# RaghuvirJonnagiri/LatticeBoltzmannSimulations

Hardware: AMD Instinct MI355X
Metric: MLUPS (million lattice updates/sec) D2Q9 MRT cavity (higher is better)
Workload: dtype f32

## Files before the change

### latticeboltzmannsimulations_amd/csrc/lbm_stream.hpp

```cpp
#pragma once
#include "lbm_kernels.hpp"

constexpr int ST_WAVES = 16;
constexpr int ST_NT = ST_WAVES * 64;
constexpr int ST_MAX_S = ST_WAVES / 2;
constexpr int ST_LDS_BYTES = ST_WAVES * 9 * 1024;

__device__ __forceinline__ int dpp_from_lower(int v) { return __builtin_amdgcn_update_dpp(v, v, 0x138, 0xf, 0xf, false); }
__device__ __forceinline__ int dpp_from_upper(int v) { return __builtin_amdgcn_update_dpp(v, v, 0x130, 0xf, 0xf, false); }
__device__ __forceinline__ float lane_lower(float v) { return __builtin_bit_cast(float, dpp_from_lower(__builtin_bit_cast(int, v))); }
__device__ __forceinline__ float lane_upper(float v) { return __builtin_bit_cast(float, dpp_from_upper(__builtin_bit_cast(int, v))); }
__device__ __forceinline__ double lane_lower(double v) {
    const long long b = __builtin_bit_cast(long long, v);
    const unsigned lo = (unsigned)dpp_from_lower((int)(unsigned)b), hi = (unsigned)dpp_from_lower((int)(unsigned)(b >> 32));
    return __builtin_bit_cast(double, (long long)(((unsigned long long)hi << 32) | lo));
}
__device__ __forceinline__ double lane_upper(double v) {
    const long long b = __builtin_bit_cast(long long, v);
    const unsigned lo = (unsigned)dpp_from_upper((int)(unsigned)b), hi = (unsigned)dpp_from_upper((int)(unsigned)(b >> 32));
    return __builtin_bit_cast(double, (long long)(((unsigned long long)hi << 32) | lo));
}

__device__ __forceinline__ float lane_lower_e(float v, float edge) {
    return __builtin_bit_cast(float, __builtin_amdgcn_update_dpp(__builtin_bit_cast(int, edge), __builtin_bit_cast(int, v), 0x138, 0xf, 0xf, false));
}
__device__ __forceinline__ float lane_upper_e(float v, float edge) {
    return __builtin_bit_cast(float, __builtin_amdgcn_update_dpp(__builtin_bit_cast(int, edge), __builtin_bit_cast(int, v), 0x130, 0xf, 0xf, false));
}
__device__ __forceinline__ double lane_lower_e(double v, double edge) {
    const long long b = __builtin_bit_cast(long long, v), e = __builtin_bit_cast(long long, edge);
    const unsigned lo = (unsigned)__builtin_amdgcn_update_dpp((int)(unsigned)e, (int)(unsigned)b, 0x138, 0xf, 0xf, false);
    const unsigned hi = (unsigned)__builtin_amdgcn_update_dpp((int)(unsigned)(e >> 32), (int)(unsigned)(b >> 32), 0x138, 0xf, 0xf, false);
    return __builtin_bit_cast(double, (long long)(((unsigned long long)hi << 32) | lo));
}
__device__ __forceinline__ double lane_upper_e(double v, double edge) {
    const long long b = __builtin_bit_cast(long long, v), e = __builtin_bit_cast(long long, edge);
    const unsigned lo = (unsigned)__builtin_amdgcn_update_dpp((int)(unsigned)e, (int)(unsigned)b, 0x130, 0xf, 0xf, false);
    const unsigned hi = (unsigned)__builtin_amdgcn_update_dpp((int)(unsigned)(e >> 32), (int)(unsigned)(b >> 32), 0x130, 0xf, 0xf, false);
    return __builtin_bit_cast(double, (long long)(((unsigned long long)hi << 32) | lo));
}
template <typename R, int V>
__device__ __forceinline__ typename VecT<R, V>::type shift_from_lower_e(typename VecT<R, V>::type own, R edge) {
    typename VecT<R, V>::type r;
    r[0] = lane_lower_e(own[V - 1], edge);
#pragma unroll
    for (int c = 1; c < V; ++c) r[c] = own[c - 1];
    return r;
}
template <typename R, int V>
__device__ __forceinline__ typename VecT<R, V>::type shift_from_upper_e(typename VecT<R, V>::type own, R edge) {
    typename VecT<R, V>::type r;
#pragma unroll
    for (int c = 0; c < V - 1; ++c) r[c] = own[c + 1];
    r[V - 1] = lane_upper_e(own[0], edge);
    return r;
}

template <typename R, int V>
__device__ __forceinline__ typename VecT<R, V>::type shift_from_lower(typename VecT<R, V>::type own) {
    typename VecT<R, V>::type r;
    r[0] = lane_lower(own[V - 1]);
#pragma unroll
    for (int c = 1; c < V; ++c) r[c] = own[c - 1];
    return r;
}
template <typename R, int V>
__device__ __forceinline__ typename VecT<R, V>::type shift_from_upper(typename VecT<R, V>::type own) {
    typename VecT<R, V>::type r;
#pragma unroll
    for (int c = 0; c < V - 1; ++c) r[c] = own[c + 1];
    r[V - 1] = lane_upper(own[0]);
    return r;
}

__host__ __device__ constexpr int stream_rim(int S, int V) { return (S + V - 1) / V * V; }

#ifdef LBM_EXPERIMENT_NO_BARRIER
__device__ __forceinline__ void lds_barrier() { asm volatile("s_waitcnt lgkmcnt(0)" ::: "memory"); }
#else
__device__ __forceinline__ void lds_barrier() { asm volatile("s_waitcnt lgkmcnt(0)\n\ts_barrier" ::: "memory"); }
#endif

template <typename R, int V, bool PROM = false>
__device__ __forceinline__ void wall_row_rules(typename VecT<R, V>::type (&in)[Q], typename VecT<R, V>::type& rw, bool lid, R uLB, bool wl, bool wr,
                                               R& kl, R& kr) {
    typedef typename VecT<R, V>::type T;
    if (lid) {
        const T ux = T(uLB), uy = T((R)0);
        const T cq = (R)1.5 * (ux * ux + uy * uy);
        auto fek = [&](int k) {
            const T cu = cu_of<T>(k, ux, uy);
            if constexpr (PROM) {
                const T rt = rw * weight<R>(k), usqr = ux * ux + uy * uy;
                T fe;
#pragma unroll
                for (int c = 0; c < V; ++c) fe[c] = feq_prom(rt[c], cu[c], usqr[c]);
                return fe;
            } else {
                return (rw * weight<R>(k)) * ((((R)1. + (R)3.0 * cu) + ((R)4.5 * cu) * cu) - cq);
            }
        };
        if (wl) {
            const R g7 = kl;
            in[1][0] = (fek(1)[0] - fek(3)[0]) + in[3][0];
            in[5][0] = (fek(5)[0] - fek(7)[0]) + g7;
            in[8][0] = (fek(8)[0] - fek(6)[0]) + in[6][0];
        }
        if (wr) {
            const R g8 = kr;
            in[3][V - 1] = (-fek(1)[V - 1] + fek(3)[V - 1]) + in[1][V - 1];
            in[6][V - 1] = (-fek(8)[V - 1] + fek(6)[V - 1]) + g8;
            in[7][V - 1] = (-fek(5)[V - 1] + fek(7)[V - 1]) + in[5][V - 1];
        }
        in[4] = (-fek(2) + fek(4)) + in[2];
        in[7] = (-fek(5) + fek(7)) + in[5];
        in[8] = (-fek(6) + fek(8)) + in[6];
        if (wl) kl = in[7][0];
        if (wr) kr = in[8][V - 1];
        rw = ((in[0] + in[1]) + in[3]) + (R)2. * ((in[2] + in[5]) + in[6]);
    } else {
        if (wl) {
            const R g6 = kl;
            in[1][0] = (R)0 + in[3][0];
            in[5][0] = (R)0 + in[7][0];
            in[8][0] = (R)0 + g6;
        }
        if (wr) {
            const R g5 = kr;
            in[3][V - 1] = (R)0 + in[1][V - 1];
            in[6][V - 1] = (R)0 + in[8][V - 1];
            in[7][V - 1] = (R)0 + g5;
        }
        in[2] = (R)0 + in[4];
        in[5] = (R)0 + in[7];
        in[6] = (R)0 + in[8];
        if (wl) kl = in[6][0];
        if (wr) kr = in[5][V - 1];
    }
}

template <typename R, int V, bool WALLS>
__device__ __forceinline__ void build_in(typename VecT<R, V>::type (&in)[Q], typename VecT<R, V>::type o0, typename VecT<R, V>::type o1,
                                         typename VecT<R, V>::type o3, typename VecT<R, V>::type u2, typename VecT<R, V>::type u5,
                                         typename VecT<R, V>::type u6, typename VecT<R, V>::type d4, typename VecT<R, V>::type d7,
                                         typename VecT<R, V>::type d8) {
    in[0] = o0;
    in[2] = u2;
    in[4] = d4;
    if (WALLS) {
        in[1] = shift_from_lower_e<R, V>(o1, (R)0 + o3[1]);
        in[5] = shift_from_lower_e<R, V>(u5, (R)0 + d7[1]);
        in[8] = shift_from_lower_e<R, V>(d8, (R)0 + u6[1]);
        in[3] = shift_from_upper_e<R, V>(o3, (R)0 + o1[V - 2]);
        in[6] = shift_from_upper_e<R, V>(u6, (R)0 + d8[V - 2]);
        in[7] = shift_from_upper_e<R, V>(d7, (R)0 + u5[V - 2]);
    } else {
        in[1] = shift_from_lower<R, V>(o1);
        in[5] = shift_from_lower<R, V>(u5);
        in[8] = shift_from_lower<R, V>(d8);
        in[3] = shift_from_upper<R, V>(o3);
        in[6] = shift_from_upper<R, V>(u6);
        in[7] = shift_from_upper<R, V>(d7);
    }
}

template <typename R, int COLL, bool TURB, bool WALLS = false, bool SLAB = false>
__device__ __forceinline__ void stream_segment(const R* __restrict__ src, R* __restrict__ dst, const Geo& geo, const Relax<R>& w, R* __restrict__ lds,
                                               int S, int xs, int ya, int yb, int xe, int own_lo = 0, int own_hi = 0) {
    constexpr int V = 16 / (int)sizeof(R), ROW = 64 * V;
    typedef typename VecT<R, V>::type T;
    const int wv = __builtin_amdgcn_readfirstlane((int)(threadIdx.x >> 6)), lane = threadIdx.x & 63;
    const int q = ((wv & 7) << 1) | (wv >> 3);
    const int RV = stream_rim(S, V) / V;
    const bool wall_lo = WALLS && (!SLAB || geo.y0 == 0), wall_hi = WALLS && (!SLAB || geo.y0 + geo.ny == geo.NY);
    const int y_first = wall_lo ? max(ya - (S - 1), 0) : ya - (S - 1);
    const int y_end = wall_hi ? min(yb + (S - 1), geo.ny) : yb + (S - 1);
    const int y_lid = wall_lo ? 0 : -(1 << 30), y_bot = wall_hi ? geo.ny - 1 : -(1 << 30);
    const int nb = y_end - y_first;
    const int x0 = xs + lane * V;
    const bool lane_in = x0 < geo.nx;
    const bool lane_out = WALLS ? (x0 >= own_lo && x0 < own_hi) : (lane >= RV && lane < 64 - RV && x0 < xe);
    const bool wl = WALLS && x0 == 0, wr = WALLS && x0 + V == geo.nx;
    const bool side_strip = WALLS && (xs == 0 || xs + ROW >= geo.nx);
    const bool narrow = WALLS && xs + ROW > geo.nx;
    R* const slot_mine = lds + (q * 9) * ROW;
    R* const up_mine = slot_mine + lane * V;
    const R* const up_below = lds + (((q + 1) & (ST_WAVES - 1)) * 9) * ROW + lane * V;
    const R* const down_above = lds + (((q + ST_WAVES - 1) & (ST_WAVES - 1)) * 9 + 3) * ROW + lane * V;

    T in[Q], outv[Q], hq, hr;
#ifdef LBM_EXP_NO_HBM
    auto row_base = [&](const R* p, int k, int y) { return (const char*)(p + ((long long)k * geo.plane + (long long)((y & 63) + GHY) * geo.row)); };
#else
    auto row_base = [&](const R* p, int k, int y) { return (const char*)(p + ((long long)k * geo.plane + (long long)(y + GHY) * geo.row)); };
#endif
    const unsigned lane_off = (unsigned)(GH + x0) * (unsigned)sizeof(R);
    auto cell = [&](const char* base, int dx) {
        unsigned off = lane_off;
        asm volatile("" : "+v"(off));
        return (const R*)(base + (off + (unsigned)(dx * (int)sizeof(R))));
    };
    const unsigned lane_off_ld = WALLS ? (unsigned)(GH + min(x0, max(geo.nx - V, 0))) * (unsigned)sizeof(R) : lane_off;
    auto cell_ld = [&](const char* base, int dx) {
        unsigned off = lane_off_ld;
        asm volatile("" : "+v"(off));
        return (const R*)(base + (off + (unsigned)(dx * (int)sizeof(R))));
    };
    auto load_row = [&](int y, bool exists) {
        if (WALLS) {
            if (exists) {
#pragma unroll
                for (int k = 0; k < Q; ++k) in[k] = vload<R, V, false>(cell_ld(row_base(src, k, y + cyk(k)), -cxk(k)), cxk(k) == 0);
                if (TURB) {
                    hq = vload<R, V, false>(cell_ld(row_base(src, K_QEQ, y), 0), true);
                    hr = vload<R, V, false>(cell_ld(row_base(src, K_RHO, y), 0), true);
                }
            } else {
#pragma unroll
                for (int k = 0; k < Q; ++k) in[k] = T{};
                hq = hr = T{};
            }
            return;
        }
        if (!lane_in || !exists) return;
#pragma unroll
        for (int k = 0; k < Q; ++k) in[k] = vload<R, V, false>(cell(row_base(src, k, y + cyk(k)), -cxk(k)), cxk(k) == 0);
        if (TURB) {
            hq = vload<R, V, false>(cell(row_base(src, K_QEQ, y), 0), true);
            hr = vload<R, V, false>(cell(row_base(src, K_RHO, y), 0), true);
        }
    };
    auto post = [&](int level, bool up, bool down) __attribute__((always_inline)) {
        R* const dn = up_mine + (3 + (level & 1) * 3) * ROW;
        const T p2 = outv[2], p5 = outv[5], p6 = outv[6], p4 = outv[4], p7 = outv[7], p8 = outv[8];
#ifdef LBM_EXP_NO_LDS
        if (geo.nx < 0)
#endif
        if (up) {
            *reinterpret_cast<T*>(up_mine) = p2;
            *reinterpret_cast<T*>(up_mine + ROW) = p5;
            *reinterpret_cast<T*>(up_mine + 2 * ROW) = p6;
        }
#ifdef LBM_EXP_NO_LDS
        if (geo.nx < 0)
#endif
        if (down) {
            *reinterpret_cast<T*>(dn) = p4;
            *reinterpret_cast<T*>(dn + ROW) = p7;
            *reinterpret_cast<T*>(dn + 2 * ROW) = p8;
        }
    };
    auto block = [&](int b, auto wrow_tag) __attribute__((always_inline)) {
        constexpr bool WROW = decltype(wrow_tag)::value;
        const int y = y_first + b;
        const bool wrow = WALLS && WROW, lid = WALLS && WROW && y == 0;
        R* const st = slot_mine + (lid ? 0 : 3 * ROW);
        auto update = [&](bool first) {
            int kind = 0;
            T rw = T{};
            R kl = (R)0, kr = (R)0;
            if (WALLS) {
                if constexpr (WROW) {
                    if (first) {
                        if (lid) rw = vload<R, V, false>(cell_ld(row_base(src, 0, -1), 0), true);
                        kl = lid ? in[7][0] : in[6][0];
                        kr = lid ? in[8][V - 1] : in[5][V - 1];
                    } else {
                        if (lid) rw = *reinterpret_cast<const T*>(st + lane * V);
                        kl = st[ROW + lane];
                        kr = st[2 * ROW + lane];
                    }
                    wall_row_rules<R, V, coll_is_prom(COLL)>(in, rw, lid, w.uLB, wl, wr, kl, kr);
                    kind = lid ? 1 : 2;
                } else if (side_strip && (first || narrow)) {
                    if (wl && first) { in[1][0] = (R)0 + in[3][0]; in[5][0] = (R)0 + in[7][0]; in[8][0] = (R)0 + in[6][0]; }
                    if (wr) { in[3][V - 1] = (R)0 + in[1][V - 1]; in[6][V - 1] = (R)0 + in[8][V - 1]; in[7][V - 1] = (R)0 + in[5][V - 1]; }
                }
            }
#ifdef LBM_EXP_NO_COLLIDE
#pragma unroll
            for (int k = 0; k < Q; ++k) outv[k] = in[k];
#else
            collide_vec<R, COLL, V, TURB>(in, w, outv, hq, hr, wl && kind == 0, wr && kind == 0, kind);
#endif
            if constexpr (WALLS && WROW) {
                if (lid) *reinterpret_cast<T*>(st + lane * V) = rw;
                st[ROW + lane] = kl;
                st[2 * ROW + lane] = kr;
            }
        };
        const bool up = !lid, down = !(wrow && !lid);
        update(true);
        if (S > 1) post(1, up, down);
        lds_barrier();
        lds_barrier();
        for (int l = 1; l < S; ++l) {
            const R* const dn = down_above + (l & 1) * 3 * ROW;
#ifdef LBM_EXP_NO_LDS
            build_in<R, V, WALLS>(in, outv[0], outv[1], outv[3], outv[2], outv[5], outv[6], outv[4], outv[7], outv[8]);
#else
            build_in<R, V, WALLS>(in, outv[0], outv[1], outv[3], *reinterpret_cast<const T*>(up_below), *reinterpret_cast<const T*>(up_below + ROW),
                                  *reinterpret_cast<const T*>(up_below + 2 * ROW), *reinterpret_cast<const T*>(dn), *reinterpret_cast<const T*>(dn + ROW),
                                  *reinterpret_cast<const T*>(dn + 2 * ROW));
#endif
            update(false);
            if (l + 1 < S) {
                post(l + 1, up, down);
                lds_barrier();
                lds_barrier();
            }
        }
        {
            const T hq_done = hq, hr_done = hr;
            T rw_done = T{};
            R kl_done = (R)0, kr_done = (R)0;
            if (WALLS && wrow) {
                if (lid) rw_done = *reinterpret_cast<const T*>(st + lane * V);
                kl_done = st[ROW + lane];
                kr_done = st[2 * ROW + lane];
            }
            if (lane_out && y >= ya && y < yb) {
#pragma unroll
                for (int k = 0; k < Q; ++k) vstore<R, V, false>(const_cast<R*>(cell(row_base(dst, k, y), 0)), outv[k]);
                if (TURB) {
                    vstore<R, V, false>(const_cast<R*>(cell(row_base(dst, K_QEQ, y), 0)), hq_done);
                    vstore<R, V, false>(const_cast<R*>(cell(row_base(dst, K_RHO, y), 0)), hr_done);
                }
                if (WALLS && wrow) {
                    if (lid) {
                        vstore<R, V, false>(const_cast<R*>(cell(row_base(dst, 0, -1), 0)), rw_done);
                        if (wl) *const_cast<R*>(cell(row_base(dst, 7, -1), 1)) = kl_done;
                        if (wr) *const_cast<R*>(cell(row_base(dst, 8, -1), V - 2)) = kr_done;
                    } else {
                        if (wl) *const_cast<R*>(cell(row_base(dst, 6, geo.ny), 1)) = kl_done;
                        if (wr) *const_cast<R*>(cell(row_base(dst, 5, geo.ny), V - 2)) = kr_done;
                    }
                }
            }
            if (S > 1) lds_barrier();
            load_row(y_first + b + ST_WAVES, b + ST_WAVES < nb);
            if (S > 1) lds_barrier();
        }
        for (int i = 2 * S; i < ST_WAVES; ++i) lds_barrier();
    };
#pragma unroll
    for (int k = 0; k < Q; ++k) in[k] = T{};
    hq = T{}; hr = T{};
    for (int i = 0; i < q; ++i) lds_barrier();
    load_row(y_first + q, q < nb);
    for (int b = q; b < nb; b += ST_WAVES) {
        const int y = y_first + b;
        if (WALLS && (SLAB ? (y == y_lid || y == y_bot) : (y == 0 || y == geo.ny - 1))) block(b, std::true_type{});
        else block(b, std::false_type{});
    }
}

template <typename R, int COLL, int SEM, bool TURB>
__global__ __launch_bounds__(ST_NT) void k_stream(const R* __restrict__ src, R* __restrict__ dst, Geo geo, Relax<R> w, int S, int F, int xe, int ye,
                                                  int nstrips, int H, FramePtrs<R> fp, int nframe, int nsegx, int nsegy, int seg, int use_lds,
                                                  int lo, int hi, int bands, int xcd_bands) {
    __shared__ __align__(16) R lds[ST_LDS_BYTES / sizeof(R)];
    if ((int)blockIdx.x < nframe) {
        frame_passes<R, COLL, SEM, TURB, ST_NT>(fp, 0, geo, w, F, S, nsegx, nsegy, lo, hi, (int)blockIdx.x, seg, use_lds ? lds : nullptr, bands);
        return;
    }
    constexpr int V = 16 / (int)sizeof(R);
    int b = blockIdx.x - nframe;
    if (xcd_bands) {
        const int per = ((int)gridDim.x - nframe) >> 3;
        if (b < (per << 3)) b = (b & 7) * per + (b >> 3);
    }
    const int strip = b % nstrips, sy = b / nstrips;
    const int R_ = stream_rim(S, V);
    const int xs = F - R_ + strip * (64 * V - 2 * R_);
    int ya, yb;
    if (bands) {
        const bool top = (bands & 1) && sy == 0;
        if (top) { ya = -(lo > 0 ? lo - 1 : 0); yb = F; }
        else { ya = geo.ny - F; yb = geo.ny + (hi > 0 ? hi - 1 : 0); }
    } else {
        ya = F + sy * H; yb = min(ye, ya + H);
    }
    if (ya >= yb) return;
    stream_segment<R, COLL, TURB>(src, dst, geo, w, lds, S, xs, ya, yb, xe);
}

__host__ __device__ constexpr int stream_walls_strips(int nx, int S, int V) {
    return nx <= 64 * V ? 1 : (nx - 64 * V + (64 * V - 2 * stream_rim(S, V)) - 1) / (64 * V - 2 * stream_rim(S, V)) + 1;
}
template <int V>
__device__ __forceinline__ void walls_strip(const Geo& geo, int S, int strip, int nstrips, int& xs, int& own_lo, int& own_hi) {
    const int R_ = stream_rim(S, V), TXu = 64 * V - 2 * R_;
    xs = min(strip * TXu, max(geo.nx - 64 * V, 0));
    own_lo = strip == 0 ? 0 : strip * TXu + R_;
    own_hi = strip == nstrips - 1 ? geo.nx : (strip + 1) * TXu + R_;
}

template <typename R, int COLL, bool TURB>
__global__ __launch_bounds__(ST_NT) void k_stream_walls(const R* __restrict__ src, R* __restrict__ dst, Geo geo, Relax<R> w, int S, int nstrips, int H,
                                                        int xcd_bands) {
    __shared__ __align__(16) R lds[ST_LDS_BYTES / sizeof(R)];
    constexpr int V = 16 / (int)sizeof(R);
    const int b = xcd_bands ? xcd_band(blockIdx.x, gridDim.x) : (int)blockIdx.x;
    const int strip = b % nstrips, sy = b / nstrips;
    int xs, own_lo, own_hi;
    walls_strip<V>(geo, S, strip, nstrips, xs, own_lo, own_hi);
    const int ya = sy * H, yb = min(geo.ny, ya + H);
    if (ya >= yb) return;
    stream_segment<R, COLL, TURB, true>(src, dst, geo, w, lds, S, xs, ya, yb, 0, own_lo, own_hi);
}
template <typename R, int COLL, bool TURB>
__global__ __launch_bounds__(ST_NT) void k_stream_walls_slab(const R* __restrict__ src, R* __restrict__ dst, Geo geo, Relax<R> w, int S, int nstrips, int H,
                                                             int xcd_bands, int ybeg, int yend, int bands, int lo, int hi, int F) {
    __shared__ __align__(16) R lds[ST_LDS_BYTES / sizeof(R)];
    constexpr int V = 16 / (int)sizeof(R), W = 64 * V;
    int b = blockIdx.x;
    if (xcd_bands) {
        const int per = (int)gridDim.x >> 3;
        if (b < (per << 3)) b = (b & 7) * per + (b >> 3);
    }
    const int strip = b % nstrips, sy = b / nstrips;
    const int R_ = stream_rim(S, V), TXu = W - 2 * R_;
    const int xs = min(strip * TXu, max(geo.nx - W, 0));
    const int own_lo = strip == 0 ? 0 : strip * TXu + R_;
    const int own_hi = strip == nstrips - 1 ? geo.nx : (strip + 1) * TXu + R_;
    int ya, yb;
    if (bands) {
        const bool top = (bands & 1) && sy == 0;
        if (top) { ya = -(lo > 0 ? lo - 1 : 0); yb = F; }
        else { ya = geo.ny - F; yb = geo.ny + (hi > 0 ? hi - 1 : 0); }
    } else {
        ya = ybeg + sy * H; yb = min(yend, ya + H);
    }
    if (ya >= yb) return;
    stream_segment<R, COLL, TURB, true, true>(src, dst, geo, w, lds, S, xs, ya, yb, 0, own_lo, own_hi);
}

constexpr int SP_MAX_WAVES = 12;
constexpr int SP_NT = SP_MAX_WAVES * 64;

constexpr int SP_MAX_S = SP_MAX_WAVES - 2;
constexpr int SP_SLOTS = 12;
constexpr int SP_LDS_BYTES = SP_MAX_WAVES * SP_SLOTS * 1024;

template <typename R, int COLL, bool TURB>
__device__ __forceinline__ void stream_pairs_segment(const R* __restrict__ src, R* __restrict__ dst, const Geo& geo, const Relax<R>& w, R* __restrict__ lds,
                                                     int S, int xs, int ya, int yb, int own_lo, int own_hi) {
    constexpr int V = 16 / (int)sizeof(R), ROW = 64 * V;
    typedef typename VecT<R, V>::type T;
    const int W = (int)(blockDim.x >> 6);
    const int wv = __builtin_amdgcn_readfirstlane((int)(threadIdx.x >> 6)), lane = threadIdx.x & 63;
    const int y_first = max(ya - (S - 1), 0), y_end = min(yb + (S - 1), geo.ny);
    const int nb = y_end - y_first, npairs = (nb + 1) >> 1;
    const int x0 = xs + lane * V;
    const bool lane_out = x0 >= own_lo && x0 < own_hi;
    const bool wl = x0 == 0, wr = x0 + V == geo.nx;
    const bool side_strip = xs == 0 || xs + ROW >= geo.nx;
    const bool narrow = xs + ROW > geo.nx;
    R* const slot_mine = lds + (wv * SP_SLOTS) * ROW;
    R* const post_mine = slot_mine + lane * V;
    const R* const up_below = lds + (((wv + 1 == W ? 0 : wv + 1)) * SP_SLOTS) * ROW + lane * V;
    const R* const down_above = lds + (((wv == 0 ? W - 1 : wv - 1)) * SP_SLOTS + 3) * ROW + lane * V;

    T in[Q], outv[Q], rawB[Q];
    T a0, a1, a3, a4, a7, a8, b0, b1, b3, b2, b5, b6;
    T hqA, hrA, hqB, hrB;
    auto row_base = [&](const R* p, int k, int y) __attribute__((always_inline)) { return (const char*)(p + ((long long)k * geo.plane + (long long)(y + GHY) * geo.row)); };
    const unsigned lane_off = (unsigned)(GH + x0) * (unsigned)sizeof(R);
    auto cell = [&](const char* base, int dx) __attribute__((always_inline)) {
        unsigned off = lane_off;
        asm volatile("" : "+v"(off));
        return (const R*)(base + (off + (unsigned)(dx * (int)sizeof(R))));
    };
    const unsigned lane_off_ld = (unsigned)(GH + min(x0, max(geo.nx - V, 0))) * (unsigned)sizeof(R);
    auto cell_ld = [&](const char* base, int dx) __attribute__((always_inline)) {
        unsigned off = lane_off_ld;
        asm volatile("" : "+v"(off));
        return (const R*)(base + (off + (unsigned)(dx * (int)sizeof(R))));
    };
    auto load_pair = [&](int j) __attribute__((always_inline)) {
        if (j < npairs) {
            const int yA = y_first + 2 * j, yB = yA + 1;
#pragma unroll
            for (int k = 0; k < Q; ++k) in[k] = vload<R, V, false>(cell_ld(row_base(src, k, yA + cyk(k)), -cxk(k)), cxk(k) == 0);
            if (TURB) {
                hqA = vload<R, V, false>(cell_ld(row_base(src, K_QEQ, yA), 0), true);
                hrA = vload<R, V, false>(cell_ld(row_base(src, K_RHO, yA), 0), true);
            }
            const int yBc = min(yB, y_end - 1);
#pragma unroll
            for (int k = 0; k < Q; ++k) rawB[k] = vload<R, V, false>(cell_ld(row_base(src, k, yBc + cyk(k)), -cxk(k)), cxk(k) == 0);
            if (TURB) {
                hqB = vload<R, V, false>(cell_ld(row_base(src, K_QEQ, yBc), 0), true);
                hrB = vload<R, V, false>(cell_ld(row_base(src, K_RHO, yBc), 0), true);
            }
        } else {
#pragma unroll
            for (int k = 0; k < Q; ++k) { in[k] = T{}; rawB[k] = T{}; }
            hqA = hrA = hqB = hrB = T{};
        }
    };
    auto park_B = [&]() __attribute__((always_inline)) {
#pragma unroll
        for (int k = 0; k < Q; ++k) *reinterpret_cast<T*>(post_mine + (3 + k) * ROW) = rawB[k];
    };
    auto update = [&](int y, bool first, T& hq, T& hr, auto wp_tag) __attribute__((always_inline)) {
        constexpr bool WP = decltype(wp_tag)::value;
        int kind = 0;
        if constexpr (WP) {
            const bool wrow = y == 0 || y == geo.ny - 1, lid = y == 0;
            R* const st = slot_mine + (lid ? 0 : 3 * ROW);
            T rw = T{};
            R kl = (R)0, kr = (R)0;
            if (wrow) {
                if (first) {
                    if (lid) rw = vload<R, V, false>(cell_ld(row_base(src, 0, -1), 0), true);
                    kl = lid ? in[7][0] : in[6][0];
                    kr = lid ? in[8][V - 1] : in[5][V - 1];
                } else {
                    if (lid) rw = *reinterpret_cast<const T*>(st + lane * V);
                    kl = st[ROW + lane];
                    kr = st[2 * ROW + lane];
                }
                wall_row_rules<R, V, coll_is_prom(COLL)>(in, rw, lid, w.uLB, wl, wr, kl, kr);
                kind = lid ? 1 : 2;
                if (lid) *reinterpret_cast<T*>(st + lane * V) = rw;
                st[ROW + lane] = kl;
                st[2 * ROW + lane] = kr;
            }
        }
        if (kind == 0 && side_strip && (first || narrow)) {
            if (wl && first) { in[1][0] = (R)0 + in[3][0]; in[5][0] = (R)0 + in[7][0]; in[8][0] = (R)0 + in[6][0]; }
            if (wr) { in[3][V - 1] = (R)0 + in[1][V - 1]; in[6][V - 1] = (R)0 + in[8][V - 1]; in[7][V - 1] = (R)0 + in[5][V - 1]; }
        }
        collide_vec<R, COLL, V, TURB>(in, w, outv, hq, hr, wl && kind == 0, wr && kind == 0, kind);
    };
    auto store_row = [&](int y, const T& hq, const T& hr) __attribute__((always_inline)) {
        if (!(lane_out && y >= ya && y < yb)) return;
#pragma unroll
        for (int k = 0; k < Q; ++k) vstore<R, V, false>(const_cast<R*>(cell(row_base(dst, k, y), 0)), outv[k]);
        if (TURB) {
            vstore<R, V, false>(const_cast<R*>(cell(row_base(dst, K_QEQ, y), 0)), hq);
            vstore<R, V, false>(const_cast<R*>(cell(row_base(dst, K_RHO, y), 0)), hr);
        }
        if (y == 0 || y == geo.ny - 1) {
            const bool lid = y == 0;
            const R* const st = slot_mine + (lid ? 0 : 3 * ROW);
            const R kl = st[ROW + lane], kr = st[2 * ROW + lane];
            if (lid) {
                vstore<R, V, false>(const_cast<R*>(cell(row_base(dst, 0, -1), 0)), *reinterpret_cast<const T*>(st + lane * V));
                if (wl) *const_cast<R*>(cell(row_base(dst, 7, -1), 1)) = kl;
                if (wr) *const_cast<R*>(cell(row_base(dst, 8, -1), V - 2)) = kr;
            } else {
                if (wl) *const_cast<R*>(cell(row_base(dst, 6, geo.ny), 1)) = kl;
                if (wr) *const_cast<R*>(cell(row_base(dst, 5, geo.ny), V - 2)) = kr;
            }
        }
    };
#pragma unroll
    for (int k = 0; k < Q; ++k) { in[k] = T{}; rawB[k] = T{}; }
    hqA = hrA = hqB = hrB = T{};
    a0 = a1 = a3 = a4 = a7 = a8 = b0 = b1 = b3 = b2 = b5 = b6 = T{};
    const int rounds = (npairs + W - 1) / W;
    const int total = 2 * W * rounds + 2 * W;
    int done = 2 * wv;
    load_pair(wv);
    for (int i = 0; i < 2 * wv; ++i) {
        if (i == 2) park_B();
        lds_barrier();
    }
    if (2 * wv <= 2) park_B();
    auto pair_body = [&](int j, auto wp_tag) __attribute__((always_inline)) {
        const int yA = y_first + 2 * j, yB = yA + 1;
        const bool lidA = yA == 0, botB = yB >= geo.ny - 1;
        auto after_A = [&](int l1) __attribute__((always_inline)) {
            a0 = outv[0]; a1 = outv[1]; a3 = outv[3]; a4 = outv[4]; a7 = outv[7]; a8 = outv[8];
            const T p2 = outv[2], p5 = outv[5], p6 = outv[6];
            if (l1 < S) {
                if (!lidA) {
                    *reinterpret_cast<T*>(post_mine) = p2;
                    *reinterpret_cast<T*>(post_mine + ROW) = p5;
                    *reinterpret_cast<T*>(post_mine + 2 * ROW) = p6;
                }
            } else {
                store_row(yA, hqA, hrA);
            }
            lds_barrier();
        };
        auto after_B = [&](int l1) __attribute__((always_inline)) {
            b0 = outv[0]; b1 = outv[1]; b3 = outv[3]; b2 = outv[2]; b5 = outv[5]; b6 = outv[6];
            const T p4 = outv[4], p7 = outv[7], p8 = outv[8];
            if (l1 < S) {
                if (!botB) {
                    R* const dn = post_mine + (3 + (l1 & 1) * 3) * ROW;
                    *reinterpret_cast<T*>(dn) = p4;
                    *reinterpret_cast<T*>(dn + ROW) = p7;
                    *reinterpret_cast<T*>(dn + 2 * ROW) = p8;
                }
            }
            lds_barrier();
        };
        update(yA, true, hqA, hrA, wp_tag);
        after_A(1);
#pragma unroll
        for (int k = 0; k < Q; ++k) in[k] = *reinterpret_cast<const T*>(post_mine + (3 + k) * ROW);
        update(yB, true, hqB, hrB, wp_tag);
        after_B(1);
        for (int l = 1; l < S; ++l) {
            {
                const R* const dn = down_above + (l & 1) * 3 * ROW;
                build_in<R, V, true>(in, a0, a1, a3, b2, b5, b6, *reinterpret_cast<const T*>(dn), *reinterpret_cast<const T*>(dn + ROW),
                                     *reinterpret_cast<const T*>(dn + 2 * ROW));
                *reinterpret_cast<T*>(post_mine + 9 * ROW) = a4;
                *reinterpret_cast<T*>(post_mine + 10 * ROW) = a7;
                *reinterpret_cast<T*>(post_mine + 11 * ROW) = a8;
                update(yA, false, hqA, hrA, wp_tag);
                after_A(l + 1);
            }
            {
                build_in<R, V, true>(in, b0, b1, b3, *reinterpret_cast<const T*>(up_below), *reinterpret_cast<const T*>(up_below + ROW),
                                     *reinterpret_cast<const T*>(up_below + 2 * ROW), *reinterpret_cast<const T*>(post_mine + 9 * ROW),
                                     *reinterpret_cast<const T*>(post_mine + 10 * ROW), *reinterpret_cast<const T*>(post_mine + 11 * ROW));
                update(yB, false, hqB, hrB, wp_tag);
                after_B(l + 1);
            }
        }
        {
            const T hq_done = hqB, hr_done = hrB;
            load_pair(j + W);
            store_row(yB, hq_done, hr_done);
        }
    };
    for (int j = wv; j < npairs; j += W) {
        const int yA = y_first + 2 * j;
        if (yA == 0 || yA + 1 >= geo.ny - 1) pair_body(j, std::true_type{});
        else pair_body(j, std::false_type{});
        for (int i = 2 * S; i < 2 * W; ++i) {
            if (i == 2 * S + 2) park_B();
            lds_barrier();
        }
        done += 2 * W;
    }
    for (; done < total; ++done) lds_barrier();
}

template <typename R, int COLL, bool TURB>
__global__ __launch_bounds__(SP_NT) void k_stream_pairs(const R* __restrict__ src, R* __restrict__ dst, Geo geo, Relax<R> w, int S, int nstrips, int H,
                                                        int xcd_bands) {
    __shared__ __align__(16) R lds[SP_LDS_BYTES / sizeof(R)];
    constexpr int V = 16 / (int)sizeof(R);
    const int b = xcd_bands ? xcd_band(blockIdx.x, gridDim.x) : (int)blockIdx.x;
    const int strip = b % nstrips, sy = b / nstrips;
    int xs, own_lo, own_hi;
    walls_strip<V>(geo, S, strip, nstrips, xs, own_lo, own_hi);
    const int ya = sy * H, yb = min(geo.ny, ya + H);
    if (ya >= yb) return;
    stream_pairs_segment<R, COLL, TURB>(src, dst, geo, w, lds, S, xs, ya, yb, own_lo, own_hi);
}
```

Before: 380,300.

## Skip unneeded temporal-blocking levels per row and specialize side-strip wall paths

Computes per-row the number of useful fused time levels (nupd) from the row's distance to the owned y-range and skips collide/stream work for levels that cannot affect owned output, still issuing matching barriers. Adds a compile-time SIDE specialization so interior strips drop wall checks, unrolls levels by two for the wall non-turbulent case, and changes DPP to bound_ctrl zero-fill. It also recomputes lane/x0 inside the block and pins scalars in SGPRs via asm barriers to steer register allocation. The risk is extra code size, more register pressure, and subtle barrier-count mismatches if nupd logic is wrong.

After: 377,100. Within noise of the previous version (-0.8%).

```diff
diff --git a/latticeboltzmannsimulations_amd/csrc/lbm_stream.hpp b/latticeboltzmannsimulations_amd/csrc/lbm_stream.hpp
--- a/latticeboltzmannsimulations_amd/csrc/lbm_stream.hpp
+++ b/latticeboltzmannsimulations_amd/csrc/lbm_stream.hpp
@@ -6,8 +6,8 @@
 constexpr int ST_MAX_S = ST_WAVES / 2;
 constexpr int ST_LDS_BYTES = ST_WAVES * 9 * 1024;
 
-__device__ __forceinline__ int dpp_from_lower(int v) { return __builtin_amdgcn_update_dpp(v, v, 0x138, 0xf, 0xf, false); }
-__device__ __forceinline__ int dpp_from_upper(int v) { return __builtin_amdgcn_update_dpp(v, v, 0x130, 0xf, 0xf, false); }
+__device__ __forceinline__ int dpp_from_lower(int v) { return __builtin_amdgcn_update_dpp(0, v, 0x138, 0xf, 0xf, true); }
+__device__ __forceinline__ int dpp_from_upper(int v) { return __builtin_amdgcn_update_dpp(0, v, 0x130, 0xf, 0xf, true); }
 __device__ __forceinline__ float lane_lower(float v) { return __builtin_bit_cast(float, dpp_from_lower(__builtin_bit_cast(int, v))); }
 __device__ __forceinline__ float lane_upper(float v) { return __builtin_bit_cast(float, dpp_from_upper(__builtin_bit_cast(int, v))); }
 __device__ __forceinline__ double lane_lower(double v) {
@@ -179,8 +179,7 @@
     const int nb = y_end - y_first;
     const int x0 = xs + lane * V;
     const bool lane_in = x0 < geo.nx;
-    const bool lane_out = WALLS ? (x0 >= own_lo && x0 < own_hi) : (lane >= RV && lane < 64 - RV && x0 < xe);
-    const bool wl = WALLS && x0 == 0, wr = WALLS && x0 + V == geo.nx;
+    const bool lane_out_frame = !WALLS && lane >= RV && lane < 64 - RV && x0 < xe;
     const bool side_strip = WALLS && (xs == 0 || xs + ROW >= geo.nx);
     const bool narrow = WALLS && xs + ROW > geo.nx;
     R* const slot_mine = lds + (q * 9) * ROW;
@@ -250,10 +249,22 @@
             *reinterpret_cast<T*>(dn + 2 * ROW) = p8;
         }
     };
-    auto block = [&](int b, auto wrow_tag) __attribute__((always_inline)) {
+    auto multi = [&]() __attribute__((always_inline)) {
+        int s = S;
+        asm volatile("" : "+s"(s));
+        return s > 1;
+    };
+    auto block = [&](int b, auto wrow_tag, auto side_tag) __attribute__((always_inline)) {
         constexpr bool WROW = decltype(wrow_tag)::value;
+        constexpr bool SIDE = WALLS && decltype(side_tag)::value;
         const int y = y_first + b;
+        const int nupd = S - max(max(ya - y, y - yb + 1), 0);
         const bool wrow = WALLS && WROW, lid = WALLS && WROW && y == 0;
+        unsigned lo_b = lane_off;
+        asm volatile("" : "+v"(lo_b));
+        const int x0 = (int)(lo_b / (unsigned)sizeof(R)) - GH, lane = (int)((unsigned)(x0 - xs) / (unsigned)V);
+        const bool wl = SIDE && x0 == 0, wr = SIDE && x0 + V == geo.nx;
+        const bool lane_out = WALLS ? (x0 >= own_lo && x0 < own_hi) : lane_out_frame;
         R* const st = slot_mine + (lid ? 0 : 3 * ROW);
         auto update = [&](bool first) {
             int kind = 0;
@@ -270,9 +281,11 @@
                         kl = st[ROW + lane];
                         kr = st[2 * ROW + lane];
                     }
-                    wall_row_rules<R, V, coll_is_prom(COLL)>(in, rw, lid, w.uLB, wl, wr, kl, kr);
+                    R u_lid = w.uLB;
+                    asm volatile("" : "+s"(u_lid));
+                    wall_row_rules<R, V, coll_is_prom(COLL)>(in, rw, lid, u_lid, wl, wr, kl, kr);
                     kind = lid ? 1 : 2;
-                } else if (side_strip && (first || narrow)) {
+                } else if (SIDE && (first || narrow)) {
                     if (wl && first) { in[1][0] = (R)0 + in[3][0]; in[5][0] = (R)0 + in[7][0]; in[8][0] = (R)0 + in[6][0]; }
                     if (wr) { in[3][V - 1] = (R)0 + in[1][V - 1]; in[6][V - 1] = (R)0 + in[8][V - 1]; in[7][V - 1] = (R)0 + in[5][V - 1]; }
                 }
@@ -291,24 +304,38 @@
         };
         const bool up = !lid, down = !(wrow && !lid);
         update(true);
-        if (S > 1) post(1, up, down);
+        if (multi()) post(1, up, down);
         lds_barrier();
         lds_barrier();
-        for (int l = 1; l < S; ++l) {
+        auto level = [&](int l, bool more) __attribute__((always_inline)) {
             const R* const dn = down_above + (l & 1) * 3 * ROW;
 #ifdef LBM_EXP_NO_LDS
-            build_in<R, V, WALLS>(in, outv[0], outv[1], outv[3], outv[2], outv[5], outv[6], outv[4], outv[7], outv[8]);
+            build_in<R, V, SIDE>(in, outv[0], outv[1], outv[3], outv[2], outv[5], outv[6], outv[4], outv[7], outv[8]);
 #else
-            build_in<R, V, WALLS>(in, outv[0], outv[1], outv[3], *reinterpret_cast<const T*>(up_below), *reinterpret_cast<const T*>(up_below + ROW),
-                                  *reinterpret_cast<const T*>(up_below + 2 * ROW), *reinterpret_cast<const T*>(dn), *reinterpret_cast<const T*>(dn + ROW),
-                                  *reinterpret_cast<const T*>(dn + 2 * ROW));
+            build_in<R, V, SIDE>(in, outv[0], outv[1], outv[3], *reinterpret_cast<const T*>(up_below), *reinterpret_cast<const T*>(up_below + ROW),
+                                 *reinterpret_cast<const T*>(up_below + 2 * ROW), *reinterpret_cast<const T*>(dn), *reinterpret_cast<const T*>(dn + ROW),
+                                 *reinterpret_cast<const T*>(dn + 2 * ROW));
 #endif
             update(false);
-            if (l + 1 < S) {
+            if (more) {
                 post(l + 1, up, down);
                 lds_barrier();
                 lds_barrier();
             }
+        };
+        int l = 1;
+        if constexpr (WALLS && !TURB) {
+            for (; l + 1 < nupd; l += 2) {
+                level(l, true);
+                level(l + 1, l + 2 < S);
+            }
+            if (l < nupd) level(l, l + 1 < S);
+        } else {
+            for (; l < nupd; ++l) level(l, l + 1 < S);
+        }
+        for (int i = nupd; i + 1 < S; ++i) {
+            lds_barrier();
+            lds_barrier();
         }
         {
             const T hq_done = hq, hr_done = hr;
@@ -337,9 +364,9 @@
                     }
                 }
             }
-            if (S > 1) lds_barrier();
+            if (multi()) lds_barrier();
             load_row(y_first + b + ST_WAVES, b + ST_WAVES < nb);
-            if (S > 1) lds_barrier();
+            if (multi()) lds_barrier();
         }
         for (int i = 2 * S; i < ST_WAVES; ++i) lds_barrier();
     };
@@ -350,8 +377,9 @@
     load_row(y_first + q, q < nb);
     for (int b = q; b < nb; b += ST_WAVES) {
         const int y = y_first + b;
-        if (WALLS && (SLAB ? (y == y_lid || y == y_bot) : (y == 0 || y == geo.ny - 1))) block(b, std::true_type{});
-        else block(b, std::false_type{});
+        if (WALLS && (SLAB ? (y == y_lid || y == y_bot) : (y == 0 || y == geo.ny - 1))) block(b, std::true_type{}, std::true_type{});
+        else if (side_strip) block(b, std::false_type{}, std::true_type{});
+        else block(b, std::false_type{}, std::false_type{});
     }
 }
 
```
